# sevagh/umx.cpp

Hardware: AMD Instinct MI355X
Metric: realtime-factor (audio-sec/wall-sec) UMX-L 4-stem, 60 s seg (higher is better)
Workload: dtype f32 (activations as 2 x fp16 planes of the power-of-two-scaled row, integer weights exact in fp16, f32 accumulate on the fp16 matrix cores; fp32-grade: 1.4-2.2x the error of an fp32 evaluation, profiles/r06_v2_accuracy_vs_float64.txt)

## Files before the change

umx.cpp_amd/__init__.py:

```python
import ctypes as C
import os
import subprocess
from pathlib import Path

import numpy as np

from . import ggml

HERE = Path(__file__).resolve().parent
ROOT = HERE.parent
NB, CROP, KX, NOUT, NFFT, HOP = 2049, 1487, 2976, 4098, 4096, 1024
SEGMENT_SAMPLES = 60 * 44100

UMX_OK, ERR_ARG, ERR_HIP, ERR_MODEL, ERR_TIMEOUT, ERR_NODEVICE = 0, 1, 2, 3, 4, 5
DTYPE_F32, DTYPE_U8, DTYPE_U16 = 0, 1, 2
FLAG_NO_WIENER = 0x1
FLAG_LSTM_STEPWISE = 0x10
FLAG_DEBUG_TAPS = 0x20
FLAG_LSTM_FORCE_SAFE = 0x40
FLAG_LSTM_PROFILE = 0x80
FLAG_PRECISE_ACT = 0x1000
FLAG_DEBUG_LSTM_ABORT = 0x2000
FLAG_RESIDUAL = 0x8000
FLAG_RESET_SEGMENTS = 0x4000
# ... 468 lines not shown
            k += 1
        return res

    def infer_batch_ptrs(self, audio_ptrs, ns, out_ptrs, flags=0, where="device"):
        nb = len(audio_ptrs)
        aud = (C.c_void_p * nb)(*[p or None for p in audio_ptrs])
        n_ = (C.c_int * nb)(*ns)
        outs = (C.c_void_p * (4 * nb))(*[p or None for p in out_ptrs])
        fn = self.lib.umx_hip_infer_batch_device if where == "device" else self.lib.umx_hip_infer_batch_async
        self._check(fn(self.h, nb, aud, n_, outs, flags))

    def infer_segment_device(self, audio_ptr, n, out_ptrs, flags=0):
        arr = (C.c_void_p * 4)(*out_ptrs)
        self._check(self.lib.umx_hip_infer_segment_device(self.h, C.c_void_p(audio_ptr), n, arr, flags))

    def sync(self):
        self._check(self.lib.umx_hip_sync(self.h))

    def last_error(self):
        return self.lib.umx_hip_last_error(self.h).decode()

    def lstm_was_persistent(self):
        return bool(self.lib.umx_hip_lstm_was_persistent(self.h))

    def lstm_mode(self):
        return self.lib.umx_hip_lstm_mode(self.h)

    def lstm_profile(self):
        buf = (C.c_ulonglong * 48)()
        self._check(self.lib.umx_hip_debug_lstm_profile(self.h, buf))
        a = np.array(buf[:], dtype=np.uint64).reshape(3, 2, 8)
        return a

    def gemm_kernel_name(self, mode):
        return self.lib.umx_hip_gemm_kernel_name(self.h, mode).decode()

    def lstm_kernel_name(self):
        return self.lib.umx_hip_lstm_kernel_name(self.h).decode()

    def lstm_placement(self, n=256):
        buf = (C.c_ulonglong * n)()
        self._check(self.lib.umx_hip_debug_lstm_placement(self.h, buf, n))
        a = np.array(buf[:], dtype=np.uint64)
        return [(int(v >> 48) & 15, int(v >> 40) & 255, int(v >> 32) & 255, int(v) & 0xffffffff) for v in a]

    def tap(self, what, target=0):
        n = self.lib.umx_hip_read_tap(self.h, what.encode(), target, None, 0)
        if n < 0:
            raise UmxError(ERR_ARG, f"tap {what!r} unavailable ({n})")
        buf = np.empty(n, np.float32)
        got = self.lib.umx_hip_read_tap(self.h, what.encode(), target, buf.ctypes.data_as(_fp), n)
        if got != n:
            raise UmxError(ERR_HIP, f"tap {what!r} failed ({got})")
        T, H = self.T, self.hidden
        what = what.split("@")[0].split("#")[0]
        if what in ("lstm_l0", "lstm_l1"):
            return buf.reshape(T, H)
        if what == "proj":
            return buf.reshape(T, 4 * H)
        if what in ("spec", "y"):
            return buf.view(np.complex64).reshape(2, T, NB)
        if what in ("mix_mag", "target_mag"):
            return buf.reshape(2, T, NB)
        if what == "x":
            return buf.reshape(T, KX)
        if what in ("fc1", "lstm", "fc2"):
# ... 348 lines not shown
```

umx.cpp_amd/csrc/engine.hip:

```cpp
#include "../../include/umx_hip.h"
#include <chrono>
#include <dlfcn.h>

#include <algorithm>
#include <numeric>
#include <cmath>
#include <cstdio>
#include <cstdlib>
#include <cstring>
#include <map>
#include <mutex>
#include <string>
#include <vector>

#include "common.h"
#include "gemm_bf16x3.h"
#include "gemm_planes.h"
#include "gemm_planes_pp.h"
#include "gemm_planes_ps.h"
#include "lstm_kernels.h"
#include "lstm_batch.h"
#include "lstm_batch8.h"
#include "track_kernels.h"
#include "resample.h"
// ... 227 lines not shown
    else if (ev)
        g.pool.push_back(ev);
    return e;
}
}

static const void *lstm_persistent_fn(int kpw, bool precise)
{
    return precise ? (kpw == 8    ? reinterpret_cast<const void *>(lstm_persistent_kernel<8, true>)
                      : kpw == 16 ? reinterpret_cast<const void *>(lstm_persistent_kernel<16, true>)
                      : kpw == 32 ? reinterpret_cast<const void *>(lstm_persistent_kernel<32, true>)
                                  : reinterpret_cast<const void *>(lstm_persistent_kernel<64, true>))
                   : (kpw == 8    ? reinterpret_cast<const void *>(lstm_persistent_kernel<8, false>)
                      : kpw == 16 ? reinterpret_cast<const void *>(lstm_persistent_kernel<16, false>)
                      : kpw == 32 ? reinterpret_cast<const void *>(lstm_persistent_kernel<32, false>)
                                  : reinterpret_cast<const void *>(lstm_persistent_kernel<64, false>));
}
template <int HL> static const void *lstm_batch_fn_hl(bool wq, bool precise)
{
    return wq ? (precise ? reinterpret_cast<const void *>(lstm_batch_kernel<HL, true, true>)
                         : reinterpret_cast<const void *>(lstm_batch_kernel<HL, true, false>))
              : (precise ? reinterpret_cast<const void *>(lstm_batch_kernel<HL, false, true>)
                         : reinterpret_cast<const void *>(lstm_batch_kernel<HL, false, false>));
}
#ifndef UMX_FUSE_LSTM_PLANES
#define UMX_FUSE_LSTM_PLANES 1
#endif
template <int HL> static const void *lstm_batch8_fn_hl(bool precise, int no)
{
    if (no == 2)
        return precise ? reinterpret_cast<const void *>(lstm_batch8_kernel<HL, true, 2>) : reinterpret_cast<const void *>(lstm_batch8_kernel<HL, false, 2>);
    return precise ? reinterpret_cast<const void *>(lstm_batch8_kernel<HL, true, 1>) : reinterpret_cast<const void *>(lstm_batch8_kernel<HL, false, 1>);
}
static const void *lstm_batch8_fn(int Hl, bool precise, int no = 1)
{
    return Hl == 512 ? lstm_batch8_fn_hl<512>(precise, no) : Hl == 256 ? lstm_batch8_fn_hl<256>(precise, no) : nullptr;
}
static const void *lstm_batch_fn(int Hl, bool wq, bool precise)
{
    switch (Hl)
    {
    case 64: return lstm_batch_fn_hl<64>(wq, precise);
    case 128: return lstm_batch_fn_hl<128>(wq, precise);
    case 256: return lstm_batch_fn_hl<256>(wq, precise);
    case 512: return lstm_batch_fn_hl<512>(wq, precise);
    default: return nullptr;
    }
}

struct GemmKernel
{
    const void *fn = nullptr;
    int lds = 0;
};
template <class K> static const void *kernel_ptr(K *k) { return reinterpret_cast<const void *>(k); }

template <int MODE> static GemmKernel bx_kernel_m(int bq)
{
    if (bq == BQ_F32)
        return {kernel_ptr(gemm_bf16x3_kernel<MODE, BQ_F32>), BX_LDS_BYTES};
    if constexpr (MODE == G_FC1 || MODE == G_IH)
    {
        if (bq == BQ_U8X)
            return {kernel_ptr(gemm_bf16x3_kernel<MODE, BQ_U8X>), BX_LDS_BYTES};
        if (bq == BQ_U8)
            return {kernel_ptr(gemm_bf16x3_kernel<MODE, BQ_U8>), BX_LDS_BYTES};
    }
    else if (bq == BQ_U16)
// ... 120 lines not shown
        void *q = nullptr;
        UMX_HIP_CHECK(hipMalloc(&q, std::max<size_t>(count, 1) * sizeof(T_)));
        allocs.push_back(q);
        if (zero)
            UMX_HIP_CHECK(hipMemset(q, 0, std::max<size_t>(count, 1) * sizeof(T_)));
        *p = reinterpret_cast<T_ *>(q);
        return UMX_OK;
    }
    template <class T_> int upload(T_ **p, const std::vector<T_> &h)
    {
        int rc = dalloc(p, h.size(), false);
        if (rc)
            return rc;
        UMX_HIP_CHECK(hipMemcpy(*p, h.data(), h.size() * sizeof(T_), hipMemcpyHostToDevice));
        return UMX_OK;
    }
    int init(int device_, int hidden, int segment_samples, const umx_tensor_view *tensors, int n_tensors,
             unsigned create_flags, int n_tracks);
    size_t weight_bytes = 0;
    bool wiener_fused = true;
    bool gemm_planes = false;
    void launch_split(Lane &ln, int nl, hipStream_t st, int which, const int *active, int nact);
    void launch_gemm_planes(Lane &ln, int nl, hipStream_t st, int mode, int layer, const int *active, int nact, bool dbg);
    void launch_gemm_lanes(Slot &sl, hipStream_t st, int nb, const float *const *audio_dev, int mode, int layer, const int *active,
                           int nact, bool dbg);
    bool u8_dequant = false;
    unsigned char *whh_q[3] = {};
    float whh_s[3][8] = {}, whh_o[3][8] = {};
    int infer_device(const float *audio_dev, int n, float *const out[4], unsigned flags);
    int infer_batch(int nb, const float *const *audio_dev, const int *n, float *const *out , unsigned flags);
    int lstm_batch_capacity = 0;
    bool lstm_batch8_ok = false;
    int lstm8_poll_delay = 0;
    bool env_lstm8_paired = true;
    int env_lstm8_min = 1;
    bool lstm_rowsums = false;
    bool lstm_writes_planes = false;
    size_t state_floats() const { return (size_t)4 * 12 * Hl; }
    int track(const float *audio_host, int length, int shift_offset, float *const out_host[4], unsigned flags,
              void (*progress)(float, void *), void *progress_user);
    int tracks(int nt, const float *const *audio_host, const int *length, const int *shift_offset, float *const *out_host, unsigned flags,
               void (*progress)(float, void *), void *progress_user, const int *rate = nullptr);
    int tracks_once(int nt, const float *const *audio_host, const int *length, const int *shift_offset, float *const *out_host,
                    unsigned flags, void (*progress)(float, void *), void *progress_user, const int *rate);
    std::map<std::pair<int, int>, float *> rs_taps;
    int resample_plan(int rate_in, int rate_out, ResampleGeom &g, const float **taps_dev);
    struct RsStage
    {
        float *in = nullptr, *out[4] = {};
        size_t cap = 0;
    };
    std::vector<RsStage> rs_stage;
    struct TrackBufs
    {
        float *in = nullptr, *out[4] = {}, *sumw = nullptr, *seg[kMaxSlots][4] = {};
        size_t cap = 0;
    };
    std::vector<TrackBufs> trk;
    hipEvent_t trk_acc_ev[kMaxSlots] = {};
    int phase_begin(const float *audio_host, int n, unsigned flags);
    int phase_begin_device(const float *audio_dev, int n, unsigned flags);
    int phase_end_device(float *const out_dev_[4]);
    const float *ph_audio = nullptr;
    int phase_layer(int layer);
    int phase_end(float *const out_host[4]);
    int ph_next = -1;
// ... 62 lines not shown
```

umx.cpp_amd/csrc/engine_init.h:

```cpp
namespace
{
bool dequant(const umx_tensor_view &tv, size_t expect, std::vector<float> &out)
{
    size_t nel = 1;
    for (int i = 0; i < tv.n_dims; ++i)
        nel *= (size_t)tv.ne[i];
    if (nel != expect)
        return false;
    out.resize(nel);
    if (tv.dtype == UMX_DTYPE_F32)
        memcpy(out.data(), tv.data, nel * sizeof(float));
    else if (tv.dtype == UMX_DTYPE_U8)
    {
        const uint8_t *q = static_cast<const uint8_t *>(tv.data);
        for (size_t i = 0; i < nel; ++i)
            out[i] = (float)q[i] * tv.scale + tv.offset;
    }
    else if (tv.dtype == UMX_DTYPE_U16)
    {
        const uint16_t *q = static_cast<const uint16_t *>(tv.data);
        for (size_t i = 0; i < nel; ++i)
            out[i] = (float)q[i] * tv.scale + tv.offset;
    }
    else
// ... 71 lines not shown

    const bool keepq = !(create_flags & UMX_CREATE_DEQUANTISE_AT_LOAD);
    auto view = [&](int tg, const std::string &name) -> const umx_tensor_view * {
        auto it = idx[tg].find(name);
        return it == idx[tg].end() ? nullptr : it->second;
    };
    auto all_q = [&](const std::string &name, int dtype, size_t expect) {
        for (int tg = 0; tg < 4; ++tg)
        {
            const umx_tensor_view *tv = view(tg, name);
            size_t n = 1;
            for (int i = 0; tv && i < tv->n_dims; ++i)
                n *= (size_t)tv->ne[i];
            if (!keepq || !tv || tv->dtype != dtype || n != expect)
                return false;
        }
        return true;
    };

    if (create_flags & UMX_CREATE_GEMM_F32)
    {
        set_error("UMX_CREATE_GEMM_F32: the fp32-MFMA GEMM flavour was removed in round 3 (slower and, against float64, less accurate "
                  "than the split-operand kernels: profiles/r02_accuracy_vs_float64.txt)");
        return UMX_ERR_ARG;
    }
    if (const char *e = getenv("UMX_GEMM_PP"))
        env_gemm_pp = atoi(e);
    if (const char *e = getenv("UMX_GEMM_PS"))
        env_gemm_ps = atoi(e);
    if (const char *e = getenv("UMX_LSTM8_POLL_DELAY"))
        lstm8_poll_delay = atoi(e);
    if (const char *e = getenv("UMX_LSTM8_PAIRED"))
        env_lstm8_paired = atoi(e) != 0;
    if (const char *e = getenv("UMX_LSTM8_MIN_LANES"))
        env_lstm8_min = atoi(e);
    if (const char *e = getenv("UMX_LSTM_POLL_DELAY"))
        lstm_poll_delay = atoi(e);
    wiener_fused = lstm_batched;
    if (const char *e = getenv("UMX_WIENER"))
        wiener_fused = std::string(e) == "fused";
    gemm_planes = (create_flags & UMX_CREATE_GEMM_PLANES) || (lstm_batched && !(create_flags & UMX_CREATE_GEMM_STAGED));
    Tp = gemm_planes ? std::max(T, 256) : round_up(T, 128);

    const int G = 4 * Hl;
    std::vector<int> gate_row(G);
    for (int sl = 0; sl < S; ++sl)
        for (int g = 0; g < 4; ++g)
            for (int u = 0; u < 16; ++u)
                gate_row[g * Hl + sl * 16 + u] = sl * 64 + u * 4 + g;
    std::vector<int> fc3_row(NOUT);
    for (int r = 0; r < NOUT; ++r)
        fc3_row[r] = r / NBINS * MAGP + r % NBINS;
    struct WeightDesc
    {
        std::string name[2];
        int nsrc, rows, cols, dst_rows, cols_pad;
        const std::vector<int> *dst_row;
        int dtype;
    };
    WeightDesc wd[W_COUNT];
    wd[W_FC1] = {{"fc1.weight"}, 1, H, NIN, H, KX, nullptr, UMX_DTYPE_U8};
    for (int l = 0; l < 3; ++l)
        wd[W_IH0 + l] = {{"lstm.weight_ih_l" + std::to_string(l), "lstm.weight_ih_l" + std::to_string(l) + "_reverse"}, 2, G, H, G, H, &gate_row,
                         UMX_DTYPE_U8};
    wd[W_FC2] = {{"fc2.weight"}, 1, H, 2 * H, H, 2 * H, nullptr, UMX_DTYPE_U16};
    wd[W_FC3] = {{"fc3.weight"}, 1, NOUT, H, NOUT_PAD, H, &fc3_row, UMX_DTYPE_U16};
// ... 404 lines not shown
        lstm_capacity = per_cu * cus;
        if (lstm_batched)
        {
            const size_t lds_max = lstmb_lds_bytes(LSTMB_GROUP_TRACKS, 8);
            per_cu = 1 << 30;
            for (int precise = 0; precise < 2; ++precise)
                for (int wq = 0; wq < 2; ++wq)
                {
                    const void *fn = lstm_batch_fn(Hl, wq != 0, precise != 0);
                    if (!fn)
                    {
                        set_error("track batching needs hidden_size in {128, 256, 512, 1024}");
                        return UMX_ERR_ARG;
                    }
                    UMX_HIP_CHECK(hipFuncSetAttribute(fn, hipFuncAttributeMaxDynamicSharedMemorySize, (int)lds_max));
                    int v = 0;
                    UMX_HIP_CHECK(hipOccupancyMaxActiveBlocksPerMultiprocessor(&v, fn, LSTM_THREADS, lstmb_lds_bytes(B > 8 ? 16 : B > 4 ? 8 : B > 2 ? 4 : B > 1 ? 2 : 1, B > 8 ? 8 : 16)));
                    per_cu = std::min(per_cu, v);
                }
            lstm_batch8_ok = false;
            if (B >= env_lstm8_min && lstm_batch8_fn(Hl, false) && !u8_dequant && whh_q[0] && whh_q[1] && whh_q[2])
            {
                lstm_batch8_ok = true;
                int per_cu8 = 1 << 30;
                for (int precise = 0; precise < 2; ++precise)
                    for (int no = 1; no <= 2; ++no)
                    {
                        const void *fn = lstm_batch8_fn(Hl, precise != 0, no);
                        UMX_HIP_CHECK(hipFuncSetAttribute(fn, hipFuncAttributeMaxDynamicSharedMemorySize, (int)lstm8_lds_bytes(Hl, no)));
                        int v = 0;
                        UMX_HIP_CHECK(hipOccupancyMaxActiveBlocksPerMultiprocessor(&v, fn, LSTM_THREADS, lstm8_lds_bytes(Hl, no)));
                        per_cu8 = std::min(per_cu8, v);
                    }
                lstm_batch8_ok = per_cu8 >= 1 && 8 * 32 <= per_cu8 * cus;
                if (lstm_batch8_ok)
                    per_cu = per_cu8;
            }
            lstm_batch_capacity = per_cu * cus;
            lstm_rowsums = UMX_FUSE_LSTM_PLANES && gemm_planes && !u8_dequant && whh_q[0] && whh_q[1] && whh_q[2];
            lstm_writes_planes = lstm_rowsums;
        }
    }
    for (const void *fn : {reinterpret_cast<const void *>(wiener_istft_kernel<true>), reinterpret_cast<const void *>(wiener_istft_kernel<false>),
                           reinterpret_cast<const void *>(wiener_istft_v_kernel)})
        UMX_HIP_CHECK(hipFuncSetAttribute(fn, hipFuncAttributeMaxDynamicSharedMemorySize, (int)WI_LDS_BYTES));
    for (int mode = G_FC1; mode <= G_FC3; ++mode)
    {
        std::vector<GemmKernel> ks;
        for (int bq : {BQ_F32, BQ_U8, BQ_U16, BQ_U8X})
            ks.push_back(bx_kernel(mode, bq));
        for (int nbp = 1; nbp <= 2; ++nbp)
            for (int kind = 0; kind < GP_KINDS; ++kind)
                ks.push_back(gp_kernel(mode, nbp, kind));
        for (const GemmKernel &k : ks)
            if (k.fn)
                UMX_HIP_CHECK(hipFuncSetAttribute(k.fn, hipFuncAttributeMaxDynamicSharedMemorySize, k.lds));
    }
    UMX_HIP_CHECK(hipDeviceSynchronize());
    return UMX_OK;
}

int umx_hip_ctx::ensure_staging()
{
    if (stage_in[0])
        return UMX_OK;
    UMX_HIP_CHECK(hipStreamCreateWithFlags(&copy_stream, hipStreamNonBlocking));
// ... 39 lines not shown
```

umx.cpp_amd/csrc/engine_lstm.h:

```cpp
int umx_hip_ctx::run_lstm_layer(Slot &sl, int layer, const int *active, int nact, bool stepwise, unsigned long long lane_mask)
{
    if (lstm_batched)
        return run_lstm_layer_batched(sl, layer, active, nact, stepwise, lane_mask);
    hipStream_t st = sl.stream;
    LstmArgs a;
    memset(&a, 0, sizeof a);
    a.W = whh[layer];
    a.Wq = whh_q[layer];
    for (int c = 0; c < 8; ++c)
    {
        a.wsc[c] = whh_s[layer][c];
        a.wof[c] = whh_o[layer][c];
    }
    a.bhh = bhh[layer];
    a.state = state;
    a.hbuf = sl.hbuf;
    a.sync = sl.lsync;
    a.status = sl.status;
    a.prof = (last_flags & UMX_FLAG_LSTM_PROFILE) ? sl.lprof : nullptr;
    a.force_safe = (last_flags & UMX_FLAG_LSTM_FORCE_SAFE) ? 1 : 0;
    a.poll_delay = lstm_poll_delay;
    a.Hl = Hl;
    a.S = S;
    a.T = T;
// ... 100 lines not shown
    }
    a.nchains = 2 * nact;
    a.lane_mask = lane_mask;
    a.poll_delay = lstm8_poll_delay;
    const bool wq_layer = whh_q[layer] != nullptr && !u8_dequant;
    const bool fuse = lstm_rowsums && wq_layer;
    if (fuse)
    {
        const size_t rows_all = (size_t)B * Tp + Mpad;
        for (int i = 0; i < 4; ++i)
        {
            const TargetAct &b = sl.lane[0].ta[i];
            a.planes[i] = layer == 0 ? b.la_p : layer == 1 ? b.lb_p : b.cat_p;
            a.rs_dir[i] = layer == 0 ? b.rs_la : layer == 1 ? b.rs_lb : b.rs_catR;
        }
        a.ldpl = a.ldo;
        a.plane_elems = rows_all * (size_t)a.ldo;
        a.rs_rows = rows_all;
    }
    a.Tp = Tp;
    int top = 0;
    for (int ln = 0; ln < LSTMB_MAX_TRACKS; ++ln)
        if ((lane_mask >> ln) & 1ull)
            top = ln + 1;
    const bool wq = whh_q[layer] != nullptr && !u8_dequant;
    const bool octets = lstm_batch8_ok;
    const int per = octets ? LSTM8_TRACKS * lstm8_octets(Hl) : LSTMB_GROUP_TRACKS;
    const int octs = octets && env_lstm8_paired && top > per ? 2 : 1;
    const int span = per * octs, parts = (top + span - 1) / span;
    a.nbp = octets ? 16 : std::min(top, span) > 8 ? 16 : std::min(top, span) > 4 ? 8 : std::min(top, span) > 2 ? 4 : std::min(top, span) > 1 ? 2 : 1;
    a.bulk = a.nbp > 8 ? 8 : 16;
    const size_t lds = octets ? lstm8_lds_bytes(Hl, octs) : lstmb_lds_bytes(a.nbp, a.bulk);
    const void *fn = octets ? lstm_batch8_fn(Hl, last_flags & UMX_FLAG_PRECISE_ACT, octs) : lstm_batch_fn(Hl, wq, last_flags & UMX_FLAG_PRECISE_ACT);
    lstm_kernel_last = octets ? "lstm_batch8_kernel" : "lstm_batch_kernel";
    const int threads = LSTM_THREADS;
    const int Sw = octets ? 32 : S;
    const bool writes_planes = fuse && lstm_writes_planes;
    if (!writes_planes)
        for (int i = 0; i < 4; ++i)
            a.planes[i] = nullptr;
    a.write_f32 = (last_flags & UMX_FLAG_DEBUG_TAPS) ? 1 : 0;
    sl.lstm_wrote_planes[layer] = writes_planes;
    sl.lstm_rows_f32[layer] = !writes_planes || a.write_f32;
    void *kargs[] = {&a};
    auto part_on = [&](int p) {
        const unsigned long long m = span >= 64 ? ~0ull : ((1ull << span) - 1ull);
        return ((lane_mask >> (span * p)) & m) != 0;
    };
    bool persistent = !stepwise && persistent_ok && 8 * S <= lstm_batch_capacity;
    int queued = 0;
    for (int p = 0; persistent && p < parts; ++p)
    {
        if (!part_on(p))
            continue;
        a.lane_base = span * p;
        a.tag_epoch = next_tag_base() >> 12;
        const bool clear = tag_epoch == 0;
        a.t_begin = 0;
        a.t_end = T;
        a.census = 1;
        a.abort_at = ((last_flags & UMX_FLAG_DEBUG_LSTM_ABORT) && layer == 1) ? T / 2 : 0;
        UMX_HIP_CHECK(hipMemsetAsync(sl.lsync, 0, sizeof(unsigned) * (clear ? lsync_words : LSTM_SYNC_HEADER_WORDS), st));
        hipError_t e = lstm_gate_launch(device, st, 8 * S * 2, 2 * n_cus,
                                        [&] { return hipLaunchKernel(fn, dim3(8 * Sw), dim3(threads), kargs, lds, st); });
        if (e != hipSuccess)
        {
            (void)hipGetLastError();
            persistent_ok = false;
            persistent = false;
            if (queued > 0)
            {
                set_error(std::string("batched LSTM: launch of a later part of a layer refused: ") + hipGetErrorString(e));
                return UMX_ERR_HIP;
            }
        }
        else
            ++queued;
    }
    if (!persistent)
    {
        a.census = 0;
        a.abort_at = 0;
        const size_t row = (size_t)4 * Hl * sizeof(float), pitch = 3 * row, off = (size_t)layer * 4 * Hl;
        UMX_HIP_CHECK(hipMemcpy2DAsync(state_alt + off, pitch, state + off, pitch, row, (size_t)4 * B, hipMemcpyDeviceToDevice, st));
        for (int step = 0; step < T; ++step)
        {
            a.t_begin = step;
            a.t_end = step + 1;
            a.state = (step & 1) ? state_alt : state;
            a.state_out = (step & 1) ? state : state_alt;
            for (int p = 0; p < parts; ++p)
                if (part_on(p))
                {
                    a.lane_base = span * p;
                    UMX_HIP_CHECK(hipLaunchKernel(fn, dim3(2 * nact * Sw), dim3(threads), kargs, lds, st));
                }
        }
// ... 10 lines not shown
```

umx.cpp_amd/csrc/lstm_batch8.h:

```cpp
#pragma once
#include "lstm_batch.h"

namespace umx
{

constexpr int LSTM8_TRACKS = 8;
constexpr int LSTM8_UNITS = 64;
__host__ __device__ constexpr int lstm8_octets(int Hl) { return 32 / (Hl / LSTM8_UNITS); }
#define LSTM8_RETRY_SLEEP 1
#define LSTM8_OOR 0x7ffffff0

__host__ __device__ inline size_t lstm8_granule_bytes(int Hl) { return (size_t)2 * 8 * (Hl / 2) * LSTM8_TRACKS * 16; }
__host__ __device__ inline size_t lstm8_h_bytes(int Hl) { return (size_t)(Hl / 32) * 4 * 16 * 16; }
#ifndef LSTM8_STG_PITCH
#define LSTM8_STG_PITCH 72
#endif
__host__ __device__ inline size_t lstm8_lds_bytes(int Hl, int no = 1) { return (size_t)no * (2 * lstm8_h_bytes(Hl) + 2 * 8 * 8 * sizeof(float) + 2 * 8 * LSTM8_STG_PITCH * 2); }

#ifndef LSTM8_EARLY_KS
#define LSTM8_EARLY_KS 13
#endif
#ifndef LSTM8_EXPERIMENT
#define LSTM8_EXPERIMENT 0
#endif
// ... 353 lines not shown
                pc7 += (unsigned long long)(c1 - ca);
            }
        }
    }
#undef LSTM8_LDS_BARRIER
#undef LSTM8_POLL
#pragma unroll
    for (int o = 0; o < NO; ++o)
        if (lane_on[o])
        {
            if (t_end > t_begin)
            {
                const size_t fr = (size_t)(dir == 0 ? t_end - 1 : T - t_end);
                outp[o][fr * ldo] = hlast[o];
                if (plp[o])
                {
                    plp[o][fr * ldpl] = (unsigned short)(plast[o] & 0xffffu);
                    plp[o][plane_elems + fr * ldpl] = (unsigned short)(plast[o] >> 16);
                }
            }
            const size_t st = (size_t)(lane0[o] + tr) * a.state_stride;
            a.state_out[st + state_off(target, a.layer, dir, 0, HL) + U] = hlast[o];
            a.state_out[st + state_off(target, a.layer, dir, 1, HL) + U] = c[o];
        }
    if (prof && l == 0)
    {
        for (int i = 0; i < 6; ++i)
            a.prof[(a.layer * 2 + pw_idx) * 8 + i] = (t_begin == 0 ? 0ull : a.prof[(a.layer * 2 + pw_idx) * 8 + i]) + pc[i];
        a.prof[(a.layer * 2 + pw_idx) * 8 + 6] = pc6;
        a.prof[(a.layer * 2 + pw_idx) * 8 + 7] = pc7;
    }
}

template <int HL, bool PRECISE, int NO> __global__ __launch_bounds__(LSTM_THREADS, 2) void lstm_batch8_kernel(LstmBArgs a)
{
    extern __shared__ __attribute__((aligned(16))) unsigned char lstm8_smem[];
    __shared__ int s_ctl[4];
    constexpr int NSH = HL / LSTM8_UNITS, G = 32 / NSH;
    const int tid = threadIdx.x;
    if (tid == 0)
    {
        if (a.census)
            lstm_census(a.sync, a.status, 32, (int)gridDim.x, a.force_safe, s_ctl);
        else
        {
            s_ctl[2] = 0;
            s_ctl[3] = 0;
        }
    }
    __syncthreads();
    if (s_ctl[3])
        return;
    int vc, shard;
    if (s_ctl[2])
    {
        vc = s_ctl[0] * G + s_ctl[1] / NSH;
        shard = s_ctl[1] % NSH;
    }
    else
    {
        const int nch = (int)gridDim.x / (G * NSH), v = (int)blockIdx.x / NSH;
        vc = (v / nch) * 8 + v % nch;
        shard = (int)blockIdx.x % NSH;
    }
    const int octet = vc >> 3, chain = vc & 7;
    unsigned mask = (unsigned)(a.lane_mask >> (a.lane_base + LSTM8_TRACKS * octet)) & 0xffu;
    if (NO > 1)
        mask |= (unsigned)(a.lane_mask >> (a.lane_base + LSTM8_TRACKS * (octet + lstm8_octets(HL)))) & 0xffu;
    if (chain >= a.nchains || mask == 0u)
        return;
    if (s_ctl[2])
        lstm8_body<HL, true, PRECISE, NO>(a, chain, shard, octet, lstm8_smem, &s_ctl[3]);
    else
        lstm8_body<HL, false, PRECISE, NO>(a, chain, shard, octet, lstm8_smem, &s_ctl[3]);
}

}
```

Before: 38730.

## Add staggered two-octet LSTM kernel overlapping matrix and gate phases across wave groups

Adds a persistent LSTM kernel variant for Hl=512 with two octets. The two wave groups run skewed schedules: one group does the matrix-core recurrence for one octet while the other computes gates for the other octet. The aim is to hide gate-activation and cross-block polling latency behind MFMA work in the serial recurrence, and the variant is on by default. In exchange it uses extra LDS for double-buffered partial sums, adds more barriers per step, and its occupancy check can lower per-CU residency.

Result: no change. 38660 (-0.2%).

```diff
diff --git a/umx.cpp_amd/__init__.py b/umx.cpp_amd/__init__.py
--- a/umx.cpp_amd/__init__.py
+++ b/umx.cpp_amd/__init__.py
@@ -524,6 +524,11 @@
         a = np.array(buf[:], dtype=np.uint64).reshape(3, 2, 8)
         return a
 
+    def lstm_stagger_profile(self):
+        buf = (C.c_ulonglong * 96)()
+        self._check(self.lib.umx_hip_debug_lstm_placement(self.h, buf, 96))
+        return np.array(buf[:], dtype=np.uint64).reshape(3, 2, 16)
+
     def gemm_kernel_name(self, mode):
         return self.lib.umx_hip_gemm_kernel_name(self.h, mode).decode()
 
diff --git a/umx.cpp_amd/csrc/engine.hip b/umx.cpp_amd/csrc/engine.hip
--- a/umx.cpp_amd/csrc/engine.hip
+++ b/umx.cpp_amd/csrc/engine.hip
@@ -283,8 +283,12 @@
         return precise ? reinterpret_cast<const void *>(lstm_batch8_kernel<HL, true, 2>) : reinterpret_cast<const void *>(lstm_batch8_kernel<HL, false, 2>);
     return precise ? reinterpret_cast<const void *>(lstm_batch8_kernel<HL, true, 1>) : reinterpret_cast<const void *>(lstm_batch8_kernel<HL, false, 1>);
 }
-static const void *lstm_batch8_fn(int Hl, bool precise, int no = 1)
-{
+static const void *lstm_batch8_fn(int Hl, bool precise, int no = 1, bool staggered = false)
+{
+    if (staggered)
+        return Hl != 512 || no != 2 ? nullptr
+               : precise            ? reinterpret_cast<const void *>(lstm_batch8_staggered_kernel<512, true>)
+                                    : reinterpret_cast<const void *>(lstm_batch8_staggered_kernel<512, false>);
     return Hl == 512 ? lstm_batch8_fn_hl<512>(precise, no) : Hl == 256 ? lstm_batch8_fn_hl<256>(precise, no) : nullptr;
 }
 static const void *lstm_batch_fn(int Hl, bool wq, bool precise)
@@ -471,6 +475,7 @@
     int lstm_batch_capacity = 0;
     bool lstm_batch8_ok = false;
     int lstm8_poll_delay = 0;
+    bool env_lstm8_stagger = true;
     bool env_lstm8_paired = true;
     int env_lstm8_min = 1;
     bool lstm_rowsums = false;
diff --git a/umx.cpp_amd/csrc/engine_init.h b/umx.cpp_amd/csrc/engine_init.h
--- a/umx.cpp_amd/csrc/engine_init.h
+++ b/umx.cpp_amd/csrc/engine_init.h
@@ -127,6 +127,8 @@
         lstm8_poll_delay = atoi(e);
     if (const char *e = getenv("UMX_LSTM8_PAIRED"))
         env_lstm8_paired = atoi(e) != 0;
+    if (const char *e = getenv("UMX_LSTM8_STAGGER"))
+        env_lstm8_stagger = atoi(e) != 0;
     if (const char *e = getenv("UMX_LSTM8_MIN_LANES"))
         env_lstm8_min = atoi(e);
     if (const char *e = getenv("UMX_LSTM_POLL_DELAY"))
@@ -597,6 +599,14 @@
                         UMX_HIP_CHECK(hipOccupancyMaxActiveBlocksPerMultiprocessor(&v, fn, LSTM_THREADS, lstm8_lds_bytes(Hl, no)));
                         per_cu8 = std::min(per_cu8, v);
                     }
+                for (int precise = 0; precise < 2; ++precise)
+                    if (const void *fn = lstm_batch8_fn(Hl, precise != 0, 2, true))
+                    {
+                        UMX_HIP_CHECK(hipFuncSetAttribute(fn, hipFuncAttributeMaxDynamicSharedMemorySize, (int)lstm8_lds_bytes_staggered(Hl)));
+                        int v = 0;
+                        UMX_HIP_CHECK(hipOccupancyMaxActiveBlocksPerMultiprocessor(&v, fn, LSTM_THREADS, lstm8_lds_bytes_staggered(Hl)));
+                        per_cu8 = std::min(per_cu8, v);
+                    }
                 lstm_batch8_ok = per_cu8 >= 1 && 8 * 32 <= per_cu8 * cus;
                 if (lstm_batch8_ok)
                     per_cu = per_cu8;
diff --git a/umx.cpp_amd/csrc/engine_lstm.h b/umx.cpp_amd/csrc/engine_lstm.h
--- a/umx.cpp_amd/csrc/engine_lstm.h
+++ b/umx.cpp_amd/csrc/engine_lstm.h
@@ -156,6 +156,9 @@
     a.bulk = a.nbp > 8 ? 8 : 16;
     const size_t lds = octets ? lstm8_lds_bytes(Hl, octs) : lstmb_lds_bytes(a.nbp, a.bulk);
     const void *fn = octets ? lstm_batch8_fn(Hl, last_flags & UMX_FLAG_PRECISE_ACT, octs) : lstm_batch_fn(Hl, wq, last_flags & UMX_FLAG_PRECISE_ACT);
+    const void *fn_stag = octs == 2 && env_lstm8_stagger ? lstm_batch8_fn(Hl, last_flags & UMX_FLAG_PRECISE_ACT, 2, true) : nullptr;
+    const void *fn_pers = fn_stag ? fn_stag : fn;
+    const size_t lds_pers = fn_stag ? lstm8_lds_bytes_staggered(Hl) : lds;
     lstm_kernel_last = octets ? "lstm_batch8_kernel" : "lstm_batch_kernel";
     const int threads = LSTM_THREADS;
     const int Sw = octets ? 32 : S;
@@ -186,7 +189,7 @@
         a.abort_at = ((last_flags & UMX_FLAG_DEBUG_LSTM_ABORT) && layer == 1) ? T / 2 : 0;
         UMX_HIP_CHECK(hipMemsetAsync(sl.lsync, 0, sizeof(unsigned) * (clear ? lsync_words : LSTM_SYNC_HEADER_WORDS), st));
         hipError_t e = lstm_gate_launch(device, st, 8 * S * 2, 2 * n_cus,
-                                        [&] { return hipLaunchKernel(fn, dim3(8 * Sw), dim3(threads), kargs, lds, st); });
+                                        [&] { return hipLaunchKernel(fn_pers, dim3(8 * Sw), dim3(threads), kargs, lds_pers, st); });
         if (e != hipSuccess)
         {
             (void)hipGetLastError();
diff --git a/umx.cpp_amd/csrc/lstm_batch8.h b/umx.cpp_amd/csrc/lstm_batch8.h
--- a/umx.cpp_amd/csrc/lstm_batch8.h
+++ b/umx.cpp_amd/csrc/lstm_batch8.h
@@ -409,6 +409,452 @@
     }
 }
 
+#ifndef LSTM8_STAG_EARLY_KS
+#define LSTM8_STAG_EARLY_KS 13
+#endif
+#ifndef LSTM8_STAG_POLL_GATE
+#define LSTM8_STAG_POLL_GATE 1
+#endif
+#ifndef LSTM8_STAG_FRAG_AHEAD
+#define LSTM8_STAG_FRAG_AHEAD 2
+#endif
+__host__ __device__ inline size_t lstm8_lds_bytes_staggered(int Hl) { return lstm8_lds_bytes(Hl, 2) + 2 * 2 * 8 * 8 * sizeof(float); }
+constexpr int LSTM8_STAG_PROF_WORDS = 16;
+constexpr int LSTM8_STAG_PROF_BASE = 64;
+
+template <int HL, bool FAST, bool PRECISE>
+__device__ __forceinline__ void lstm8_body_staggered(const LstmBArgs &a, int chain, int shard, int octet0, unsigned char *smem, int *abort_flag)
+{
+    constexpr int NO = 2;
+    constexpr int NKS = HL / 32, KSW = NKS / 8, NLD = HL * 4 / 512, GPS = HL * 4, HB = (HL / 32) * 4 * 16 * 16, OCT = lstm8_octets(HL);
+    constexpr int EARLY = LSTM8_STAG_EARLY_KS < 0 ? 0 : (LSTM8_STAG_EARLY_KS < NKS ? LSTM8_STAG_EARLY_KS : NKS - 3);
+    constexpr int HS_KS = 3 < NKS ? 3 : NKS - 1;
+    static_assert(HL % 256 == 0 && 32 % (HL / LSTM8_UNITS) == 0 && NKS >= 8, "eight waves x 32-unit k-steps");
+    const int target = a.tmap[chain >> 1], dir = chain & 1, wchain = target * 2 + dir;
+    const int tid = threadIdx.x, w = __builtin_amdgcn_readfirstlane(tid >> 6), l = tid & 63, n = l & 15, q = l >> 4;
+    const int grp = w >> 2, wg = w & 3;
+    const int tr = n & 7, tile = n >> 3;
+    const int T = a.T, S = a.S;
+    const int U = shard * LSTM8_UNITS + w * 8 + tile * 4 + q;
+
+    unsigned char *const hl = smem;
+    float *const hsp = reinterpret_cast<float *>(smem + (size_t)NO * 2 * HB);
+    unsigned short *const stg = reinterpret_cast<unsigned short *>(smem + (size_t)NO * 2 * HB + 2 * NO * 2 * 8 * 8 * sizeof(float));
+
+    f16x8 Wf[2][NKS];
+    {
+        const unsigned char *wp[2];
+#pragma unroll
+        for (int mt = 0; mt < 2; ++mt)
+        {
+            const int ug = shard * LSTM8_UNITS + w * 8 + mt * 4 + (n >> 2);
+            wp[mt] = a.Wq + (((size_t)wchain * S + (ug >> 4)) * HL + 8 * q) * 64 + 4 * (ug & 15) + (n & 3);
+        }
+#pragma unroll
+        for (int ks = 0; ks < NKS; ++ks)
+        {
+#pragma unroll
+            for (int mt = 0; mt < 2; ++mt)
+            {
+                f16x8 hw;
+#pragma unroll
+                for (int j = 0; j < 8; ++j)
+                    hw[j] = (_Float16)((float)wp[mt][(size_t)(32 * ks + j) * 64] - 128.0f);
+                Wf[mt][ks] = hw;
+            }
+            asm volatile("" ::: "memory");
+        }
+    }
+    constexpr float HSCALE = 16384.0f;
+    const float wsc = a.wsc[wchain] * (1.0f / HSCALE), wof2 = (a.wof[wchain] + 128.0f * a.wsc[wchain]) * (1.0f / HSCALE);
+    const float4 bh = *reinterpret_cast<const float4 *>(a.bhh + ((size_t)wchain * S + (U >> 4)) * 64 + 4 * (U & 15));
+
+    const int p_tr = tid & 7, p_pair = (tid >> 3) & 3, p_q = (tid >> 5) & 3, p_ks0 = tid >> 7;
+    const int lds_w = ((p_ks0 * 4 + p_q) * 16 + p_tr) * 16 + p_pair * 4;
+    const int t_begin = a.t_begin, t_end = a.t_end;
+    const size_t ldp = (size_t)a.ldp, ldo = (size_t)a.ldo, plane_elems = a.plane_elems, ldpl = (size_t)a.ldpl;
+    const unsigned tag_hi = a.tag_epoch << 12;
+    const int gbase = chain * GPS * 16, gslot = 8 * GPS * 16;
+    const int pub_off = gbase + (((U >> 3) * 4 + ((U & 7) >> 1)) * 8 + tr) * 16;
+    gu32 *status = (gu32 *)a.status;
+
+    bool lane_on[NO], p_on[NO];
+    unsigned mask8s[NO];
+    float c[NO], hlast[NO];
+    float4 p4n[NO], p4c[NO];
+    const float *Pg0 = nullptr;
+    float *outp0 = nullptr;
+    const size_t Pg_d = (size_t)LSTM8_TRACKS * OCT * a.p_stride, outp_d = (size_t)LSTM8_TRACKS * OCT * a.out_stride;
+    __amdgpu_buffer_rsrc_t gran_rs[NO];
+    int lane0[NO];
+#pragma unroll
+    for (int o = 0; o < NO; ++o)
+    {
+        const int octet = octet0 + o * OCT;
+        lane0[o] = a.lane_base + LSTM8_TRACKS * octet;
+        const unsigned mask8 = (unsigned)(a.lane_mask >> lane0[o]) & 0xffu;
+        mask8s[o] = mask8;
+        lane_on[o] = (mask8 >> tr) & 1u;
+        p_on[o] = (mask8 >> p_tr) & 1u;
+        const size_t st = (size_t)(lane0[o] + tr) * a.state_stride;
+        c[o] = lane_on[o] ? a.state[st + state_off(target, a.layer, dir, 1, HL) + U] : 0.f;
+        hlast[o] = lane_on[o] ? a.state[st + state_off(target, a.layer, dir, 0, HL) + U] : 0.f;
+        if (o == 0)
+        {
+            Pg0 = a.P[target] + (size_t)(lane0[0] + tr) * a.p_stride + ((size_t)dir * S + (U >> 4)) * 64 + 4 * (U & 15);
+            outp0 = a.out[target] + (size_t)(lane0[0] + tr) * a.out_stride + a.col0 + dir * HL + U;
+        }
+        gran_rs[o] = __builtin_amdgcn_make_buffer_rsrc(reinterpret_cast<unsigned char *>(a.sync + LSTM_SYNC_HEADER_WORDS) + (size_t)octet * lstm8_granule_bytes(HL), 0,
+                                                       (int)lstm8_granule_bytes(HL), 0x00020000);
+        p4n[o] = p4c[o] = make_float4(0.f, 0.f, 0.f, 0.f);
+        if (lane_on[o] && t_begin < t_end)
+            p4n[o] = stream_load4(Pg0 + o * Pg_d + (size_t)(dir == 0 ? t_begin : T - 1 - t_begin) * ldp);
+        const size_t sh = (size_t)(lane0[o] + p_tr) * a.state_stride + state_off(target, a.layer, dir, 0, HL);
+#pragma unroll
+        for (int i = 0; i < NLD; ++i)
+        {
+            const int k0 = (i * 4 + p_ks0) * 32 + p_q * 8 + p_pair * 2;
+            unsigned d1 = 0u, d2 = 0u;
+            if (p_on[o])
+            {
+                const float x0 = a.state[sh + k0] * HSCALE, x1 = a.state[sh + k0 + 1] * HSCALE;
+                const _Float16 a1 = (_Float16)x0, b1 = (_Float16)x1;
+                const _Float16 a2 = (_Float16)(x0 - (float)a1), b2 = (_Float16)(x1 - (float)b1);
+                d1 = (unsigned)__builtin_bit_cast(unsigned short, a1) | ((unsigned)__builtin_bit_cast(unsigned short, b1) << 16);
+                d2 = (unsigned)__builtin_bit_cast(unsigned short, a2) | ((unsigned)__builtin_bit_cast(unsigned short, b2) << 16);
+            }
+            unsigned char *dst = hl + (size_t)(o * 2 + (t_begin & 1)) * HB + lds_w + i * 4096;
+            *reinterpret_cast<unsigned *>(dst) = d1;
+            *reinterpret_cast<unsigned *>(dst + 128) = d2;
+            if (!p_on[o])
+            {
+                unsigned char *other = hl + (size_t)(o * 2 + ((t_begin & 1) ^ 1)) * HB + lds_w + i * 4096;
+                *reinterpret_cast<unsigned *>(other) = 0u;
+                *reinterpret_cast<unsigned *>(other + 128) = 0u;
+            }
+        }
+    }
+    const __amdgpu_buffer_rsrc_t rs_rs =
+        __builtin_amdgcn_make_buffer_rsrc(a.rs_dir[target], 0, a.rs_dir[target] ? (int)((size_t)2 * a.rs_rows * 4) : 0, 0x00020000);
+    const bool rs_wave = shard == 0 && w == 0, have_planes = a.planes[target] != nullptr, rows_f32 = !have_planes || a.write_f32;
+    __builtin_amdgcn_s_waitcnt(0x0f70);
+    const bool prof = a.prof != nullptr && octet0 == 0 && chain == 0 && shard == 0 && (w == 0 || w == LSTMB_PROF_WAVE);
+    unsigned pcs[14] = {0, 0, 0, 0, 0, 0, 0, 0, 0, 0, 0, 0, 0, 0}, prof_spins = 0;
+    const f16x8 ones16 = __builtin_bit_cast(f16x8, make_uint4(0x3C003C00u, 0x3C003C00u, 0x3C003C00u, 0x3C003C00u));
+#define LSTM8_LDS_BARRIER() asm volatile("s_waitcnt lgkmcnt(0)\n\ts_barrier" ::: "memory")
+    typedef unsigned v3u32 __attribute__((ext_vector_type(3)));
+    v3u32 v[NLD];
+    const int goff0 = gbase + tid * 16;
+    int sg_off = tr * LSTM8_STG_PITCH + w * 8 + tile * 4 + q;
+    asm volatile("" : "+v"(sg_off));
+    floatx4 acc0 = {0.f, 0.f, 0.f, 0.f}, acc1 = {0.f, 0.f, 0.f, 0.f};
+    long long pt = 0;
+
+    auto poll_issue = [&](int o, int step) __attribute__((always_inline)) {
+        const bool some = p_on[o] && step > t_begin && step < t_end;
+        const int base = ((step - 1) & 1) * gslot + goff0;
+#pragma unroll
+        for (int i = 0; i < NLD; ++i)
+            v[i] = __builtin_amdgcn_raw_buffer_load_b96(gran_rs[o], some ? base + i * 512 * 16 : LSTM8_OOR, 0, 16);
+    };
+    auto top = [&](int o, int step, int pslot) __attribute__((always_inline)) {
+        if (prof)
+            pt = clock64();
+        const long long t0 = pt;
+        if (step > t_begin)
+        {
+            const unsigned want = tag_hi | (unsigned)step;
+            unsigned spins = 0;
+            auto tags_bad = [&]() {
+                unsigned bad = 0;
+#pragma unroll
+                for (int i = 0; i < NLD; ++i)
+                    bad |= v[i].x ^ want;
+                return bad;
+            };
+            bool ok = true;
+            if (p_on[o])
+                ok = tags_bad() == 0u;
+            while (!__all(ok))
+            {
+                if (++spins > LSTM_SPIN_LIMIT || ((spins & 1023u) == 0 && __hip_atomic_load(status, __ATOMIC_RELAXED, __HIP_MEMORY_SCOPE_AGENT) != 0))
+                {
+                    if (l == 0)
+                        __hip_atomic_store(status, 1u + (unsigned)step, __ATOMIC_RELAXED, __HIP_MEMORY_SCOPE_AGENT);
+                    *abort_flag = 1;
+                    break;
+                }
+                __builtin_amdgcn_s_sleep(LSTM8_RETRY_SLEEP);
+                if (p_on[o])
+                {
+#pragma unroll
+                    for (int i = 0; i < NLD; ++i)
+                        v[i] = __builtin_amdgcn_raw_buffer_load_b96(gran_rs[o], ((step - 1) & 1) * gslot + goff0 + i * 512 * 16, 0, 16);
+                    ok = tags_bad() == 0u;
+                }
+            }
+            prof_spins += spins;
+            if (prof)
+                pcs[12 + pslot / 2] += (unsigned)(clock64() - t0);
+            if (p_on[o])
+            {
+                unsigned char *const hb = hl + (size_t)(o * 2 + (step & 1)) * HB;
+#pragma unroll
+                for (int i = 0; i < NLD; ++i)
+                {
+                    *reinterpret_cast<unsigned *>(hb + lds_w + i * 4096) = v[i].y;
+                    *reinterpret_cast<unsigned *>(hb + lds_w + i * 4096 + 128) = v[i].z;
+                }
+            }
+            if (lane_on[o] && rows_f32)
+                outp0[o * outp_d + (size_t)(dir == 0 ? step - 1 : T - step) * ldo] = hlast[o];
+        }
+        p4c[o] = p4n[o];
+        if (lane_on[o] && step + 1 < t_end)
+            p4n[o] = stream_load4(Pg0 + o * Pg_d + (size_t)(dir == 0 ? step + 1 : T - 2 - step) * ldp);
+    };
+    auto slot_barrier = [&](int pslot, bool had_top) __attribute__((always_inline)) {
+        long long t1 = 0;
+        if (prof)
+        {
+            t1 = clock64();
+            if (had_top)
+                pcs[8 + pslot] += (unsigned)(t1 - pt);
+        }
+        LSTM8_LDS_BARRIER();
+        if (prof)
+        {
+            pt = clock64();
+            pcs[4 + pslot] += (unsigned)(pt - t1);
+        }
+    };
+    auto phase_end = [&](int pslot) __attribute__((always_inline)) {
+        if (prof)
+        {
+            const long long t = clock64();
+            pcs[pslot] += (unsigned)(t - pt);
+            pt = t;
+        }
+    };
+    auto stage_store = [&](int o, int step) __attribute__((always_inline)) {
+        if (LSTM8_STAGE_PLANES && have_planes && step > t_begin && w < 2)
+        {
+            const int strk = l >> 3, sgrp = l & 7;
+            if ((mask8s[o] >> strk) & 1u)
+            {
+                const uint4 val = *reinterpret_cast<const uint4 *>(stg + ((o * 2 + w) * 8 + strk) * LSTM8_STG_PITCH + sgrp * 8);
+                unsigned short *dst = a.planes[target] + (size_t)w * plane_elems + ((size_t)(lane0[o] + strk) * a.Tp + (size_t)(dir == 0 ? step - 1 : T - step)) * ldpl +
+                                      a.col0 + dir * HL + shard * LSTM8_UNITS + sgrp * 8;
+                stream_store4u(reinterpret_cast<uint4 *>(dst), val);
+            }
+        }
+    };
+    auto matrix = [&](int o, int step, int po, int pstep) __attribute__((always_inline)) {
+        const unsigned char *const hb = hl + (size_t)(o * 2 + (step & 1)) * HB;
+        float *const hs = hsp + ((grp * NO + o) * 2 + (step & 1)) * 64;
+        const unsigned char *const fb = hb + (q * 16 + n) * 16;
+        floatx4 accHa = {0.f, 0.f, 0.f, 0.f}, accHb = {0.f, 0.f, 0.f, 0.f};
+        acc0 = floatx4{0.f, 0.f, 0.f, 0.f};
+        acc1 = floatx4{0.f, 0.f, 0.f, 0.f};
+        f16x8 bf[LSTM8_STAG_FRAG_AHEAD];
+#pragma unroll
+        for (int i = 0; i < LSTM8_STAG_FRAG_AHEAD; ++i)
+            bf[i] = *reinterpret_cast<const f16x8 *>(fb + i * 1024);
+        if (LSTM8_PIN_ORDER)
+            __builtin_amdgcn_sched_barrier(0);
+#pragma unroll
+        for (int kk = 0; kk < KSW; ++kk)
+            accHa = __builtin_amdgcn_mfma_f32_16x16x32_f16(ones16, *reinterpret_cast<const f16x8 *>(fb + ((2 * wg) * KSW + kk) * 1024), accHa, 0, 0, 0);
+#pragma unroll
+        for (int kk = 0; kk < KSW; ++kk)
+            accHb = __builtin_amdgcn_mfma_f32_16x16x32_f16(ones16, *reinterpret_cast<const f16x8 *>(fb + ((2 * wg + 1) * KSW + kk) * 1024), accHb, 0, 0, 0);
+#pragma unroll
+        for (int ks = 0; ks < NKS; ++ks)
+        {
+            const f16x8 cur = bf[ks % LSTM8_STAG_FRAG_AHEAD];
+            acc0 = __builtin_amdgcn_mfma_f32_16x16x32_f16(Wf[0][ks], cur, acc0, 0, 0, 0);
+            acc1 = __builtin_amdgcn_mfma_f32_16x16x32_f16(Wf[1][ks], cur, acc1, 0, 0, 0);
+            if (ks + LSTM8_STAG_FRAG_AHEAD < NKS)
+                bf[ks % LSTM8_STAG_FRAG_AHEAD] = *reinterpret_cast<const f16x8 *>(fb + (ks + LSTM8_STAG_FRAG_AHEAD) * 1024);
+            if (LSTM8_PIN_ORDER)
+                __builtin_amdgcn_sched_barrier(0);
+            if (ks == HS_KS)
+            {
+                hs[tr * 8 + 2 * wg] = accHa[0] + __int_as_float(dpp_row_ror<8>(__float_as_int(accHa[0])));
+                hs[tr * 8 + 2 * wg + 1] = accHb[0] + __int_as_float(dpp_row_ror<8>(__float_as_int(accHb[0])));
+            }
+            if (ks == EARLY && po >= 0)
+                poll_issue(po, pstep);
+        }
+    };
+    auto gates = [&](int o, int step, int po, int pstep) __attribute__((always_inline)) {
+        const float *const hs = hsp + ((grp * NO + o) * 2 + (step & 1)) * 64;
+        const float4 ha = *reinterpret_cast<const float4 *>(hs + tr * 8), hc = *reinterpret_cast<const float4 *>(hs + tr * 8 + 4);
+        const float hp8[8] = {ha.x, ha.y, ha.z, ha.w, hc.x, hc.y, hc.z, hc.w};
+        const float Hs = tree_sum<8>(hp8);
+        if (rs_wave)
+        {
+            const int rs_row = (int)(((size_t)dir * a.rs_rows + (size_t)(lane0[o] + tr) * a.Tp) * 4);
+            __builtin_amdgcn_raw_buffer_store_b32(__float_as_uint(Hs * (1.0f / 16384.0f)), rs_rs,
+                                                  (l < 8 && lane_on[o] && step > 0) ? rs_row + (dir == 0 ? step - 1 : T - step) * 4 : LSTM8_OOR, 0, 0);
+        }
+        if (po >= 0 && LSTM8_STAG_POLL_GATE == 0)
+            poll_issue(po, pstep);
+        const float hterm = wof2 * Hs;
+        float s[4];
+#pragma unroll
+        for (int r = 0; r < 4; ++r)
+        {
+            const float mine = tile ? acc1[r] : acc0[r], theirs = tile ? acc0[r] : acc1[r];
+            const float sum = mine + __int_as_float(dpp_row_ror<8>(__float_as_int(theirs)));
+            s[r] = wsc * sum + hterm;
+        }
+        const float4 p4 = p4c[o];
+        const float pre_i = (p4.x + s[0]) + bh.x, pre_f = (p4.y + s[1]) + bh.y, pre_g = (p4.z + s[2]) + bh.z, pre_o = (p4.w + s[3]) + bh.w;
+        float i_t, f_t, g_t, o_t;
+        if (PRECISE)
+        {
+            i_t = sigmoid_ref(pre_i);
+            f_t = sigmoid_ref(pre_f);
+            g_t = tanhf(pre_g);
+            o_t = sigmoid_ref(pre_o);
+        }
+        else
+        {
+            i_t = sigmoid_hw(pre_i);
+            f_t = sigmoid_hw(pre_f);
+            g_t = tanh_hw(pre_g);
+            o_t = sigmoid_hw(pre_o);
+        }
+        const float c_t = f_t * c[o] + i_t * g_t;
+        const float h = o_t * (PRECISE ? tanhf(c_t) : tanh_hw(c_t));
+        const float hs14 = h * HSCALE;
+        const _Float16 h1 = (_Float16)hs14, h2 = (_Float16)(hs14 - (float)h1);
+        const unsigned b1 = __builtin_bit_cast(unsigned short, h1), b2 = __builtin_bit_cast(unsigned short, h2);
+        const unsigned mine12 = b1 | (b2 << 16);
+        const unsigned other12 = __builtin_amdgcn_permlane16_swap(mine12, mine12, false, false)[1];
+        if (lane_on[o])
+        {
+            c[o] = c_t;
+            hlast[o] = h;
+        }
+        if (LSTM8_STAGE_PLANES && have_planes)
+        {
+            unsigned short *sg = stg + o * 2 * 8 * LSTM8_STG_PITCH + sg_off;
+            sg[0] = (unsigned short)b1;
+            sg[8 * LSTM8_STG_PITCH] = (unsigned short)b2;
+        }
+        if (po >= 0 && LSTM8_STAG_POLL_GATE != 0)
+            poll_issue(po, pstep);
+        granule_store16<FAST>(gran_rs[o], (lane_on[o] && (q & 1) == 0) ? (step & 1) * gslot + pub_off : LSTM8_OOR,
+                              make_uint4(tag_hi | (unsigned)(step + 1), b1 | (other12 << 16), (mine12 >> 16) | (other12 & 0xffff0000u), 0u));
+    };
+
+    if (grp == 0)
+    {
+        for (int step = t_begin; step < t_end; ++step)
+        {
+            if (a.abort_at && step == a.abort_at && tid == 0)
+            {
+                __hip_atomic_store(status, 1u + (unsigned)step, __ATOMIC_RELAXED, __HIP_MEMORY_SCOPE_AGENT);
+                *abort_flag = 1;
+            }
+            top(0, step, 0);
+            slot_barrier(0, true);
+            if (*abort_flag)
+                return;
+            stage_store(0, step);
+            matrix(0, step, -1, 0);
+            phase_end(0);
+            slot_barrier(1, false);
+            gates(0, step, 1, step);
+            phase_end(1);
+            top(1, step, 2);
+            slot_barrier(2, true);
+            if (*abort_flag)
+                return;
+            stage_store(1, step);
+            matrix(1, step, -1, 0);
+            phase_end(2);
+            slot_barrier(3, false);
+            gates(1, step, 0, step + 1);
+            phase_end(3);
+        }
+        LSTM8_LDS_BARRIER();
+    }
+    else
+    {
+        for (int step = t_begin; step < t_end; ++step)
+        {
+            top(0, step, 0);
+            slot_barrier(0, true);
+            if (*abort_flag)
+                return;
+            if (step > t_begin)
+                gates(1, step - 1, -1, 0);
+            phase_end(0);
+            slot_barrier(1, false);
+            matrix(0, step, 1, step);
+            phase_end(1);
+            top(1, step, 2);
+            slot_barrier(2, true);
+            if (*abort_flag)
+                return;
+            gates(0, step, -1, 0);
+            phase_end(2);
+            slot_barrier(3, false);
+            matrix(1, step, 0, step + 1);
+            phase_end(3);
+        }
+        LSTM8_LDS_BARRIER();
+        if (t_end > t_begin)
+            gates(1, t_end - 1, -1, 0);
+    }
+#undef LSTM8_LDS_BARRIER
+#pragma unroll
+    for (int o = 0; o < NO; ++o)
+        if (lane_on[o])
+        {
+            if (t_end > t_begin)
+            {
+                const size_t fr = (size_t)(dir == 0 ? t_end - 1 : T - t_end);
+                outp0[o * outp_d + fr * ldo] = hlast[o];
+                if (a.planes[target])
+                {
+                    unsigned short *plp = a.planes[target] + (size_t)(lane0[o] + tr) * a.Tp * a.ldpl + a.col0 + dir * HL + U;
+                    const float hs14 = hlast[o] * HSCALE;
+                    const _Float16 h1 = (_Float16)hs14, h2 = (_Float16)(hs14 - (float)h1);
+                    plp[fr * ldpl] = __builtin_bit_cast(unsigned short, h1);
+                    plp[plane_elems + fr * ldpl] = __builtin_bit_cast(unsigned short, h2);
+                }
+            }
+            const size_t st = (size_t)(lane0[o] + tr) * a.state_stride;
+            a.state_out[st + state_off(target, a.layer, dir, 0, HL) + U] = hlast[o];
+            a.state_out[st + state_off(target, a.layer, dir, 1, HL) + U] = c[o];
+        }
+    if (prof && l == 0)
+    {
+        unsigned hw;
+        asm volatile("s_getreg_b32 %0, hwreg(HW_REG_HW_ID)" : "=s"(hw));
+        const int pw_idx = w == 0 ? 0 : 1;
+        unsigned long long *lock = a.prof + (a.layer * 2 + pw_idx) * 8, *out = a.prof + LSTM8_STAG_PROF_BASE + (a.layer * 2 + pw_idx) * LSTM8_STAG_PROF_WORDS;
+        const unsigned m = pcs[0] + pcs[2], g = pcs[1] + pcs[3];
+        const unsigned tops = pcs[8] + pcs[10], checks = pcs[12] + pcs[13];
+        lock[0] = tops;
+        lock[1] = grp == 0 ? m : g;
+        lock[2] = pcs[4] + pcs[5] + pcs[6] + pcs[7];
+        lock[3] = grp == 0 ? g : m;
+        lock[4] = (unsigned long long)2 * (t_end - t_begin);
+        lock[5] = prof_spins;
+        lock[6] = checks;
+        lock[7] = tops - checks;
+        for (int i = 0; i < 14; ++i)
+            out[i] = pcs[i];
+        out[14] = (unsigned long long)(t_end - t_begin);
+        out[15] = hw;
+    }
+}
+
 template <int HL, bool PRECISE, int NO> __global__ __launch_bounds__(LSTM_THREADS, 2) void lstm_batch8_kernel(LstmBArgs a)
 {
     extern __shared__ __attribute__((aligned(16))) unsigned char lstm8_smem[];
@@ -452,4 +898,36 @@
         lstm8_body<HL, false, PRECISE, NO>(a, chain, shard, octet, lstm8_smem, &s_ctl[3]);
 }
 
+template <int HL, bool PRECISE> __global__ __launch_bounds__(LSTM_THREADS, 2) void lstm_batch8_staggered_kernel(LstmBArgs a)
+{
+    extern __shared__ __attribute__((aligned(16))) unsigned char lstm8_smem[];
+    __shared__ int s_ctl[4];
+    constexpr int NSH = HL / LSTM8_UNITS, G = 32 / NSH;
+    if (threadIdx.x == 0)
+        lstm_census(a.sync, a.status, 32, (int)gridDim.x, a.force_safe, s_ctl);
+    __syncthreads();
+    if (s_ctl[3])
+        return;
+    int vc, shard;
+    if (s_ctl[2])
+    {
+        vc = s_ctl[0] * G + s_ctl[1] / NSH;
+        shard = s_ctl[1] % NSH;
+    }
+    else
+    {
+        const int nch = (int)gridDim.x / (G * NSH), v = (int)blockIdx.x / NSH;
+        vc = (v / nch) * 8 + v % nch;
+        shard = (int)blockIdx.x % NSH;
+    }
+    const int octet = vc >> 3, chain = vc & 7;
+    const unsigned mask = (unsigned)((a.lane_mask >> (a.lane_base + LSTM8_TRACKS * octet)) | (a.lane_mask >> (a.lane_base + LSTM8_TRACKS * (octet + lstm8_octets(HL))))) & 0xffu;
+    if (chain >= a.nchains || mask == 0u)
+        return;
+    if (s_ctl[2])
+        lstm8_body_staggered<HL, true, PRECISE>(a, chain, shard, octet, lstm8_smem, &s_ctl[3]);
+    else
+        lstm8_body_staggered<HL, false, PRECISE>(a, chain, shard, octet, lstm8_smem, &s_ctl[3]);
 }
+
+}
```
